# evoldoers/historian

Hardware: AMD Instinct MI355X
Metric: forward-DP cells/s (higher is better)
Workload: dtype f64; 1 GPU; batch of independent 2x2000-residue protein leaf-profile pairs, WAG, t=0.2/0.3, full (unbanded) Forward DP; scaled-probability recursion with the reference's truncation: every pairwise sum of the reference's left-nested log_sum_exp drops a term that is at most e^-10 of the other, as the reference's table does (src/logsumexp.h:45); no table, log-probabilities at the store; lpEnd within 1e-9 rel. of; pairs_per_gpu=512, pairs_total=512, parallelism=pairs farmed across 1 rank(s); RCCL broadcast of model constants only

## Files before the change

historian_amd/csrc/hx_linear.hip:

```cpp
#include <hip/hip_runtime.h>
#include <cstdlib>
#include "hx_device.h"
#include "hx_lse.h"
#include "hx_common.h"
#include "hx_policy.h"
#include "hx_kernels.h"

namespace hx {

namespace {

#define HXL_PUBLISH_LAG 16
#define HX_YL_MAX_CLS_LINEAR 64
#define HXL_EMIN (-(1 << 28))
#define HXL_RENORM_MASK 6

struct L5 { double imm, imd, idm, imi, iiw; int e; };

#define HXL_EXP_M10 4.5399929762484854e-05
__device__ __forceinline__ double trunc_sum(double a, double b) {
  const double hi = fmax_plain(a, b), lo = fmin_plain(a, b);
  const int keep = lo > hi * HXL_EXP_M10 ? __double2hiint(lo) : 0;
  return hi + __hiloint2double(keep, __double2loint(lo));
}
template <bool TRUNC> __device__ __forceinline__ double lin_acc(double m, double p, double acc) {
  if (TRUNC) return trunc_sum(acc, m * p);
  return __builtin_fma(m, p, acc);
}

__device__ __forceinline__ L5 l5_zero() { return L5{0., 0., 0., 0., 0., HXL_EMIN}; }

__device__ __forceinline__ int dpp_shr1_keep0(int old, int v) {
  return __builtin_amdgcn_update_dpp(old, v, 0x138, 0xf, 0xf, false);
}
__device__ __forceinline__ double dpp_shr1_keep0(double old, double v) {
  const int lo = __builtin_amdgcn_update_dpp(__double2loint(old), __double2loint(v), 0x138, 0xf, 0xf, false);
  const int hi = __builtin_amdgcn_update_dpp(__double2hiint(old), __double2hiint(v), 0x138, 0xf, 0xf, false);
  return __hiloint2double(hi, lo);
}
__device__ __forceinline__ L5 dpp_shr1_old(const L5& o, const L5& c) {
  return L5{dpp_shr1_keep0(o.imm, c.imm), dpp_shr1_keep0(o.imd, c.imd), dpp_shr1_keep0(o.idm, c.idm),
            dpp_shr1_keep0(o.imi, c.imi), dpp_shr1_keep0(o.iiw, c.iiw), dpp_shr1_keep0(o.e, c.e)};
}

#define HXL_LOG_ENTRIES 1536
typedef double log_entry __attribute__((ext_vector_type(2)));
__device__ __forceinline__ log_entry log_issue(double m, const HX_LDS double* ltab) {
  const double f = __builtin_amdgcn_frexp_mant(m);
  unsigned idx;
  asm("v_bfe_u32 %0, %1, 11, 11" : "=v"(idx) : "v"(__double2hiint(f)));
  return *(const HX_LDS log_entry*)((const HX_LDS char*)ltab + (idx << 4));
}
__device__ __forceinline__ double log_finish(double m, int e, log_entry ce) {
  const double f = __builtin_amdgcn_frexp_mant(m);
  const int k = __builtin_amdgcn_frexp_exp(m);
  const double r = __builtin_fma(f, ce.x, -1.0);
  double p = __builtin_fma(r, 1.0 / 3.0, -0.5);
  p = __builtin_fma(p, r, 1.0);
  const double lf = __builtin_fma(p, r, ce.y);
  return __builtin_fma((double)(e + k), 0.693147180559945309417, lf);
}
__device__ __forceinline__ double log_scaled(double m, int e, const HX_LDS double* ltab) { return log_finish(m, e, log_issue(m, ltab)); }

__device__ __forceinline__ L5 from_logs(double a, double b, double c, double d, double g) {
  const double mx = vmax(vmax(vmax(a, b), vmax(c, d)), g);
  if (!(mx > HX_NEG_INF)) return l5_zero();
  const double n = __builtin_rint(mx * 1.44269504088896340736);
  const double hi = n * 0.693147180369123816490, lo = n * 1.90821492927058770002e-10;
  L5 r;
  r.imm = exp((a - hi) - lo);
  r.imd = exp((b - hi) - lo);
  r.idm = exp((c - hi) - lo);
  r.imi = exp((d - hi) - lo);
  r.iiw = exp((g - hi) - lo);
  r.e = (int)n;
  return r;
}

struct LdsPlan { int elds, ycol, yclass, flags, zero;
                 int a0, b0, a1, stride, total; };

#define HXL_RING 64
#define HXL_STAGE 128

#define HXL_PATIENCE (1 << 22)
template <int W, bool BANDED, int PPW, int DIR, bool MULTI = false, bool TRUNC = false>
__global__ void __launch_bounds__(W * PPW * 64, 4)
k_fill_leaf_linear(const DevJob* __restrict__ jobs, const double* __restrict__ exact_tab, const double* __restrict__ log_tab,
                      const LdsPlan plan, const int n_jobs, const int groups = 1, int* const counters = nullptr) {
  static_assert(!MULTI || (!BANDED && PPW == 1 && W > 1), "several workgroups per pair: unbanded pairs, one pair per workgroup");
  static_assert(!BANDED || W == 1, "banded batches run one wavefront per pair");
  static_assert(PPW == 1 || BANDED, "several pairs per workgroup: banded batches only");
  constexpr int THREADS = W * PPW * 64, PT = W * 64;
  constexpr bool RESCHED = DIR == 0;
  constexpr int RING_ENTRIES = BANDED ? 0 : W * HXL_RING;
  typedef double d2v __attribute__((ext_vector_type(2)));
  extern __shared__ __attribute__((aligned(16))) unsigned char lds[];
  double* ltab = reinterpret_cast<double*>(lds);
  const int pair = PPW == 1 ? 0 : __builtin_amdgcn_readfirstlane((int)(threadIdx.x >> 6));
  const int tid = (int)threadIdx.x - pair * PT;
  const int G = MULTI ? groups : 1;
  const int job = MULTI ? (int)blockIdx.x / G : (int)blockIdx.x * PPW + pair;
  const int grp = MULTI ? (int)blockIdx.x % G : 0;
  const bool live = PPW == 1 || job < n_jobs;
  const DevJob& J = jobs[live ? job : 0];
  unsigned char* blk_a = lds + (pair == 0 ? plan.a0 : plan.a1 + (pair - 1) * plan.stride);
  unsigned char* blk_b = pair == 0 ? lds + plan.b0 : blk_a + (plan.stride - (RING_ENTRIES + HXL_STAGE) * 48);
  double* elds = reinterpret_cast<double*>(blk_a + plan.elds);
  unsigned* ycol = reinterpret_cast<unsigned*>(blk_a + plan.ycol);
  double* yclass = reinterpret_cast<double*>(blk_a + plan.yclass);
  volatile int* prog = reinterpret_cast<volatile int*>(blk_a + plan.flags);
  volatile int* cons = prog + W;
  volatile int* drain = cons + W;
  constexpr bool lds_words = !BANDED;
  for (int k = threadIdx.x; k < 2; k += THREADS) ltab[k] = log_tab[k];
  for (int k = 2048 + threadIdx.x; k < 2 * HXL_LOG_ENTRIES; k += THREADS) ltab[k] = log_tab[k];
  if (tid < 2 * W + 1) prog[tid] = 0;
  if (tid == 0) {
    d2v* z = reinterpret_cast<d2v*>(blk_a + plan.zero);
    z[0] = d2v{0., 0.}; z[1] = d2v{0., 0.}; z[2] = d2v{0., __hiloint2double(0, HXL_EMIN)};
  }
  {
    const int Ky1 = J.y.n_cls + 1, Kx1 = J.x.n_cls + 1;
    for (int jp = tid; jp < (lds_words ? J.n_cols + 130 : 0); jp += PT) {
      const int j = jp < 64 ? 0 : (jp - 64 >= J.n_cols ? J.n_cols - 1 : jp - 64);
      if (BANDED)
        ycol[jp] = (unsigned)J.y.ecls[j] | (J.y.pack[4 * (size_t)j + 3] < 0.0 ? 0x100u : 0u) |
                   ((J.y.flags[j] & F_EDGE) ? 0x200u : 0u) | (J.max_dist >= 0 ? (unsigned)J.y.env[j] << 10 : 0u);
      else if (DIR == 0)
        ycol[jp] = (unsigned)J.y.ecls[j] | (J.y.pack[4 * (size_t)j + 3] < 0.0 ? 0xFFFF0000u : 0u);
      else {
        const int jc = J.n_cols - 1 - j;
        ycol[jp] = (unsigned)J.y.ecls[jc + 1] | (J.y.pack[4 * (size_t)jc + 3] < 0.0 ? 0xFFFF0000u : 0u);
      }
    }
    for (int c = tid; c < Ky1; c += PT) {
      const bool real = c < J.y.n_cls;
      const int rep = real ? J.y.cls_rep[c] : 0;
      yclass[2 * c] = real ? exp(J.y.pack[4 * (size_t)rep + 1]) : 0.;
      yclass[2 * c + 1] = real ? exp(J.y.pack[4 * (size_t)rep + 2]) : 0.;
    }
    for (int e = tid; e < Kx1 * Ky1; e += PT) elds[e] = exp(J.emis_pad[e]);
  }
  __syncthreads();
  const int R = J.n_rows, Cc = J.n_cols;
  const int max_dist = J.max_dist;
  const int lane = threadIdx.x & 63, wave = PPW == 1 ? (RESCHED ? __builtin_amdgcn_readfirstlane((int)(threadIdx.x >> 6)) : (int)(threadIdx.x >> 6)) : 0;
  const int64_t plane = J.plane, ss = J.strip_stride;
  const int blk = J.blk;
  HX_GLOBAL double* __restrict__ M = as_global(DIR ? J.bwd : J.fwd);
  const HX_GLOBAL d4v* xpack = (const HX_GLOBAL d4v*)as_global(J.x.pack);
  double P[5][5];
#pragma unroll
  for (int a = 0; a < 5; ++a)
#pragma unroll
    for (int d = 0; d < 5; ++d) {
      const bool used = d == 0 || (d == 1 && a != 4) || (d == 2 && a != 3) || (d == 3 && (a == 0 || a == 3)) ||
                        (d == 4 && (a == 0 || a == 3 || a == 4));
      if (!used) { P[a][d] = 0.; continue; }
      const double pv = exp(J.T[a][d]);
      double v = __hiloint2double(__builtin_amdgcn_readfirstlane(__double2hiint(pv)), __builtin_amdgcn_readfirstlane(__double2loint(pv)));
      asm volatile("" : "+s"(v));
      P[a][d] = v;
    }
  volatile HX_LDS int* progp = (volatile HX_LDS int*)prog;
  volatile HX_LDS int* consp = (volatile HX_LDS int*)cons;
  volatile HX_LDS int* drainp = (volatile HX_LDS int*)drain;
  const HX_LDS double* lt = (const HX_LDS double*)ltab;
  HX_LDS d2v* ring_mine = (HX_LDS d2v*)blk_b + (size_t)wave * (HXL_RING * 3);
  const int n_strips = live ? (R + 63) / 64 : 0;
  const int prev_wave = (wave + W - 1) % W, next_wave = (wave + 1) % W;
  const int WT = W * G, gw = grp * W + wave;
  HX_GLOBAL int* gdrain = MULTI ? (HX_GLOBAL int*)as_global(counters + 256 * job) : nullptr;
  const int prev_grp = (grp + G - 1) % G;
  bool dead = false;
  const auto wait_drained = [&](const int need) {
    if (!MULTI) {
      while (drainp[0] < need) __builtin_amdgcn_s_sleep(1);
      asm volatile("" ::: "memory");
      return;
    }
    if (dead) return;
    int polls = 0;
    while (__builtin_amdgcn_readfirstlane(__hip_atomic_load(gdrain + prev_grp, __ATOMIC_RELAXED, __HIP_MEMORY_SCOPE_AGENT)) < need) {
      if (++polls > HXL_PATIENCE) {
        dead = true;
        if (lane == 0) __hip_atomic_store(gdrain + 255, 1, __ATOMIC_RELAXED, __HIP_MEMORY_SCOPE_AGENT);
        break;
      }
      __builtin_amdgcn_s_sleep(1);
    }
    asm volatile("" ::: "memory");
  };
  const auto publish_drained = [&](const int value) {
    if (lane != 0) return;
    if (MULTI) __hip_atomic_store(gdrain + grp, value, __ATOMIC_RELAXED, __HIP_MEMORY_SCOPE_AGENT);
    else drainp[0] = value;
  };
  HX_LDS d2v* staging = (HX_LDS d2v*)blk_b + (size_t)RING_ENTRIES * 3;
  const HX_LDS d2v* ring_prev = (const HX_LDS d2v*)blk_b + (size_t)prev_wave * (HXL_RING * 3);

  for (int s = gw; s < n_strips; s += WT) {
    const int row0 = s * 64;
    const int i0 = row0 + lane;
    const bool row_valid = i0 < R;
    double fx, f_imd, f_iiw;
    int x_wait;
    unsigned eoff;
    int env_x = 0;
    bool edge_x = true;
    {
      const int ic = row_valid ? (DIR ? R - 1 - i0 : i0) : 0;
      const d4v p = xpack[ic];
      const d4v q = DIR ? xpack[ic + 1] : p;
      fx = row_valid ? exp(q.x) : 0.;
      f_imd = row_valid ? exp(q.x + q.y) : 0.;
      f_iiw = row_valid ? exp(q.x + q.z) : 0.;
      x_wait = (row_valid && !(p.w < 0.0)) ? 0 : (1 << 29);
      eoff = (unsigned)J.x.ecls[DIR ? ic + 1 : ic] * (unsigned)(J.y.n_cls + 1);
      if (BANDED) {
        env_x = J.max_dist >= 0 ? J.x.env[ic] : 0;
        edge_x = (J.x.flags[ic] & F_EDGE) != 0 || J.max_dist < 0;
      }
    }
    L5 ca = l5_zero(), cb = l5_zero(), ua = l5_zero(), ub = l5_zero();
    const bool has_above = s > 0, has_below = s + 1 < n_strips;
    const bool wrap_in = has_above && wave == 0;
    const bool wrap_out = has_below && wave == W - 1;
    const bool ring_out = has_below && !wrap_out;
    const int above_base = ((s - 1) / WT) * Cc;
    const int my_base = (s / WT) * Cc;
    int64_t store_base = (int64_t)s * ss;
    int store_t0 = 0;
    const int nsteps = (Cc + 64) & ~1;

    auto wait_for = [&](const int cols) {
      const int need = above_base + (cols < Cc ? cols : Cc);
      while (progp[prev_wave] < need) __builtin_amdgcn_s_sleep(1);
      asm volatile("" ::: "memory");
    };
    const HX_LDS d2v* ring_above = !has_above ? (const HX_LDS d2v*)(blk_a + plan.zero) : wrap_in ? (const HX_LDS d2v*)staging : ring_prev;
    const int ring_base = (wrap_in || !has_above) ? 0 : above_base;
    const int ring_mask = !has_above ? 0 : wrap_in ? HXL_STAGE - 1 : HXL_RING - 1;
    auto ring_entry = [&](const int col) -> L5 {
      const HX_LDS d2v* q = ring_above + (size_t)((ring_base + col) & ring_mask) * 3;
      const d2v a = q[0], b = q[1], c = q[2];
      return L5{a.x, a.y, b.x, b.y, c.x, __double2loint(c.y)};
    };
    auto stage_block = [&](const int c0) {
      const int hi = (c0 + 64 < Cc) ? c0 + 64 : Cc;
      const int need = above_base + hi;
      wait_drained(need);
      const int jj = c0 + lane;
      const int64_t sl = jj < Cc ? ((BANDED && DIR == 0) ? stored_slot(J, row0 - 1, jj) : cell_slot_blk(ss, blk, row0 - 1, jj)) : -1;
      if (jj < Cc && sl < 0) {
        HX_LDS d2v* q = staging + (size_t)(jj & (HXL_STAGE - 1)) * 3;
        q[0] = d2v{0., 0.}; q[1] = d2v{0., 0.}; q[2] = d2v{0., __hiloint2double(0, HXL_EMIN)};
      }
      if (sl >= 0) {
        const double a = __hip_atomic_load(M + sl, __ATOMIC_RELAXED, __HIP_MEMORY_SCOPE_AGENT);
        const double b = __hip_atomic_load(M + plane + sl, __ATOMIC_RELAXED, __HIP_MEMORY_SCOPE_AGENT);
        const double c = __hip_atomic_load(M + 2 * plane + sl, __ATOMIC_RELAXED, __HIP_MEMORY_SCOPE_AGENT);
        const double d = __hip_atomic_load(M + 3 * plane + sl, __ATOMIC_RELAXED, __HIP_MEMORY_SCOPE_AGENT);
        const double g = __hip_atomic_load(M + 4 * plane + sl, __ATOMIC_RELAXED, __HIP_MEMORY_SCOPE_AGENT);
        L5 v = from_logs(a, b, c, d, g);
        if (BANDED && max_dist >= 0) {
          const int ia = DIR ? R - row0 : row0 - 1, ja = DIR ? Cc - 1 - jj : jj;
          int dist = J.x.env[ia] - J.y.env[ja];
          dist = dist < 0 ? -dist : dist;
          if (!(((J.x.flags[ia] | J.y.flags[ja]) & F_EDGE) || dist <= max_dist)) v = l5_zero();
        }
        HX_LDS d2v* q = staging + (size_t)(jj & (HXL_STAGE - 1)) * 3;
        q[0] = d2v{v.imm, v.imd};
        q[1] = d2v{v.idm, v.imi};
        q[2] = d2v{v.iiw, __hiloint2double(0, v.e)};
      }
      asm volatile("s_waitcnt lgkmcnt(0)" ::: "memory");
    };
    auto open_sweep = [&](const int t0) {
      if (!has_above) return;
      if (wrap_in) {
        if (t0 > 0 && (t0 & 63) == 0) stage_block(t0 - 64);
        if (t0 < Cc) stage_block(t0 & ~63);
      } else {
        wait_for(8);
      }
      const L5 b0 = ring_entry(t0), bd = ring_entry(t0 > 0 ? t0 - 1 : 0);
      if (lane == 0) {
        ua = b0;
        if (BANDED && t0 > 0) ub = bd;
      }
    };
    unsigned wnext = 0;
    const HX_GLOBAL unsigned* ywords = (const HX_GLOBAL unsigned*)as_global(DIR ? J.yword_bwd : J.yword);
    auto refill_words = [&](const int i0) {
      const unsigned v = ywords[i0 + lane];
      ycol[(i0 + lane) & 255] = v;
      asm volatile("s_waitcnt vmcnt(0) lgkmcnt(0)" ::: "memory");
    };
    auto first_words = [&](const int t0) {
      if (lds_words) { wnext = ycol[t0 + 64 - lane]; return; }
      refill_words(t0 & ~63); refill_words((t0 & ~63) + 64); refill_words((t0 & ~63) + 128);
      wnext = ycol[(t0 + 64 - lane) & 255];
    };
    auto next_word = [&](const int t) -> unsigned {
      const unsigned w = wnext;
      wnext = lds_words ? ycol[t + 65 - lane] : ycol[(t + 65 - lane) & 255];
      return w;
    };
    auto step = [&](const int t, const L5& left, L5& out, L5& u1, L5& u2, const unsigned w) {
      if (!lds_words && (t & 63) == 62) refill_words(t + 2 + 128);
      if ((t & 7) == 7 && has_above && t + 1 < Cc) {
        if (wrap_in) {
          if ((t & 63) == 63) stage_block(t + 1);
        } else {
          if (lane == 0) consp[wave] = above_base + t;
          wait_for(t + 9);
        }
      }
      const unsigned c = BANDED ? (w & 0xFFu) : (w & 0xFFFFu);
      const d2v rc = reinterpret_cast<const d2v*>(yclass)[c];
      const int y_wait = BANDED ? (int)((w & 0x100u) << 21) : (int)((w >> 16) << 13);
      const double em = elds[eoff + c];
      int E;
      if (DIR == 0) {
        double s_imm = u2.imm * P[0][0];
        s_imm = lin_acc<TRUNC>(u2.imd, P[1][0], s_imm);
        s_imm = lin_acc<TRUNC>(u2.idm, P[2][0], s_imm);
        s_imm = lin_acc<TRUNC>(u2.imi, P[3][0], s_imm);
        s_imm = lin_acc<TRUNC>(u2.iiw, P[4][0], s_imm);
        const int e_diag = u2.e;
        __builtin_amdgcn_sched_barrier(0);
        u2 = ring_entry(t + 1);
        __builtin_amdgcn_sched_barrier(0);
        double s_imd = u1.imm * P[0][1];
        double s_iiw = u1.imm * P[0][4];
        double s_idm = left.imm * P[0][2];
        double s_imi = left.imm * P[0][3];
        s_imd = lin_acc<TRUNC>(u1.imd, P[1][1], s_imd);
        s_iiw = lin_acc<TRUNC>(u1.imi, P[3][4], s_iiw);
        s_idm = lin_acc<TRUNC>(left.imd, P[1][2], s_idm);
        s_imi = lin_acc<TRUNC>(left.imi, P[3][3], s_imi);
        s_imd = lin_acc<TRUNC>(u1.idm, P[2][1], s_imd);
        s_iiw = lin_acc<TRUNC>(u1.iiw, P[4][4], s_iiw);
        s_idm = lin_acc<TRUNC>(left.idm, P[2][2], s_idm);
        s_imd = lin_acc<TRUNC>(u1.imi, P[3][1], s_imd);
        s_idm = lin_acc<TRUNC>(left.iiw, P[4][2], s_idm);
        E = left.e > u1.e ? left.e : u1.e;
        E = E > e_diag ? E : e_diag;
        int du = (u1.e - E) - y_wait, dl = (left.e - E) - x_wait, dd = e_diag - E;
        if (BANDED) {
          int dist = env_x - (int)(w >> 10);
          dist = dist < 0 ? -dist : dist;
          const int out_of_env = (edge_x || (w & 0x200u) || dist <= max_dist) ? 0 : (1 << 29);
          du -= out_of_env; dl -= out_of_env; dd -= out_of_env;
        }
        out.imd = __builtin_ldexp(s_imd * f_imd, du);
        out.iiw = __builtin_ldexp(s_iiw * f_iiw, du);
        out.idm = __builtin_ldexp(s_idm * rc.x, dl);
        out.imi = __builtin_ldexp(s_imi * rc.y, dl);
        out.imm = __builtin_ldexp(s_imm * (fx * em), dd);
      } else {
        const int e_diag = u2.e;
        const double tD = u2.imm * (fx * em);
        const double t1x = u1.imd * f_imd, t2x = u1.iiw * f_iiw;
        const double t1y = left.idm * rc.x, t2y = left.imi * rc.y;
        u2 = ring_entry(t + 1);
        E = left.e > u1.e ? left.e : u1.e;
        E = E > e_diag ? E : e_diag;
        int du = (u1.e - E) - y_wait, dl = (left.e - E) - x_wait, dd = e_diag - E;
        if (BANDED) {
          int dist = env_x - (int)(w >> 10);
          dist = dist < 0 ? -dist : dist;
          const int out_of_env = (edge_x || (w & 0x200u) || dist <= max_dist) ? 0 : (1 << 29);
          du -= out_of_env; dl -= out_of_env; dd -= out_of_env;
        }
        const double D = __builtin_ldexp(tD, dd);
        const double d1x = __builtin_ldexp(t1x, du), d2x = __builtin_ldexp(t2x, du);
        const double d1y = __builtin_ldexp(t1y, dl), d2y = __builtin_ldexp(t2y, dl);
        out.imm = lin_acc<TRUNC>(P[0][3], d2y, lin_acc<TRUNC>(P[0][2], d1y, lin_acc<TRUNC>(P[0][4], d2x, lin_acc<TRUNC>(P[0][1], d1x, P[0][0] * D))));
        out.imd = lin_acc<TRUNC>(P[1][2], d1y, lin_acc<TRUNC>(P[1][1], d1x, P[1][0] * D));
        out.idm = lin_acc<TRUNC>(P[2][2], d1y, lin_acc<TRUNC>(P[2][1], d1x, P[2][0] * D));
        out.imi = lin_acc<TRUNC>(P[3][3], d2y, lin_acc<TRUNC>(P[3][4], d2x, lin_acc<TRUNC>(P[3][1], d1x, P[3][0] * D)));
        out.iiw = lin_acc<TRUNC>(P[4][2], d1y, lin_acc<TRUNC>(P[4][4], d2x, P[4][0] * D));
      }
      out.e = E;
      if ((t & HXL_RENORM_MASK) == 0) {
        if (s == 0 && t == 0) {
          if (DIR == 0) {
            if (lane == 0) { out.imm = 1.0; out.e = 0; }
          } else if (lane == 0) {
            const double lpe = J.x.pack[4 * (size_t)R] + J.y.pack[4 * (size_t)Cc];
            out.imm = exp(lpe + J.T[0][5]); out.imd = exp(lpe + J.T[1][5]); out.idm = exp(lpe + J.T[2][5]);
            out.imi = exp(lpe + J.T[3][5]); out.iiw = exp(lpe + J.T[4][5]);
            out.e = 0;
          }
        }
        const double mx = vmax(vmax(vmax(out.imm, out.imd), vmax(out.idm, out.imi)), out.iiw);
        const int k = __builtin_amdgcn_frexp_exp(mx);
        out.imm = __builtin_ldexp(out.imm, -k);
        out.imd = __builtin_ldexp(out.imd, -k);
        out.idm = __builtin_ldexp(out.idm, -k);
        out.imi = __builtin_ldexp(out.imi, -k);
        out.iiw = __builtin_ldexp(out.iiw, -k);
        out.e = mx > 0. ? out.e + k : HXL_EMIN;
      }
      if (ring_out && t >= 63 && t - 63 < Cc) {
        const int col = t - 63;
        if ((col & 7) == 0) {
          const int need = my_base + col + 8 - HXL_RING;
          while (consp[next_wave] < need) __builtin_amdgcn_s_sleep(1);
          asm volatile("" ::: "memory");
        }
        if (lane == 63) {
          HX_LDS d2v* q = ring_mine + (size_t)((my_base + col) & (HXL_RING - 1)) * 3;
          q[0] = d2v{out.imm, out.imd};
          q[1] = d2v{out.idm, out.imi};
          q[2] = d2v{out.iiw, __hiloint2double(0, out.e)};
        }
        if ((col & 7) == 7 || col == Cc - 1) {
          asm volatile("" ::: "memory");
          if (lane == 63) progp[wave] = my_base + col + 1;
        }
      }
      u2 = dpp_shr1_old(u2, out);
    };

    int wlo[2] = {0, 0}, whi[2] = {nsteps, 0};
    if (BANDED) {
      const HX_GLOBAL int32_t* win = as_global(DIR ? J.bwd_windows : J.fwd_windows);
      if (win) {
        for (int w = 0; w < 2; ++w) {
          wlo[w] = win[4 * s + 2 * w] & ~1;
          const int h = (win[4 * s + 2 * w + 1] + 1) & ~1;
          whi[w] = h < nsteps ? h : nsteps;
        }
        if (whi[1] > wlo[1] && wlo[1] <= whi[0]) { whi[0] = whi[1] > whi[0] ? whi[1] : whi[0]; wlo[1] = whi[1] = 0; }
      }
    }
    for (int wi = 0; wi < (BANDED ? 2 : 1); ++wi) {
    if (BANDED && whi[wi] <= wlo[wi]) continue;
    const int wstart = BANDED ? wlo[wi] : 0, wend = BANDED ? whi[wi] : nsteps;
    if (BANDED) { ca = l5_zero(); cb = l5_zero(); ua = l5_zero(); ub = l5_zero(); }
    if (BANDED && DIR == 0 && J.strip_base) { store_base = J.strip_base[2 * s + wi]; store_t0 = wstart; }
    open_sweep(wstart);
    first_words(wstart);
    auto step_pair = [&](const int t) {
      if (RESCHED) {
        step(t, cb, ca, ua, ub, next_word(t));
        const log_entry ea0 = log_issue(ca.imm, lt), ea1 = log_issue(ca.imd, lt), ea2 = log_issue(ca.idm, lt),
                        ea3 = log_issue(ca.imi, lt), ea4 = log_issue(ca.iiw, lt);
        step(t + 1, ca, cb, ub, ua, next_word(t + 1));
        const log_entry eb0 = log_issue(cb.imm, lt), eb1 = log_issue(cb.imd, lt);
        __builtin_amdgcn_sched_barrier(0);
        const double l0 = log_finish(ca.imm, ca.e, ea0), l1 = log_finish(ca.imd, ca.e, ea1);
        const log_entry eb2 = log_issue(cb.idm, lt), eb3 = log_issue(cb.imi, lt);
        __builtin_amdgcn_sched_barrier(0);
        const double l2 = log_finish(ca.idm, ca.e, ea2), l3 = log_finish(ca.imi, ca.e, ea3);
        const log_entry eb4 = log_issue(cb.iiw, lt);
        __builtin_amdgcn_sched_barrier(0);
        const double l4 = log_finish(ca.iiw, ca.e, ea4);
        {
          HX_GLOBAL char* Mu = (HX_GLOBAL char*)(M + (store_base + (int64_t)((t - store_t0) >> 1) * blk));
          unsigned voff = (unsigned)lane << 4;
          asm("" : "+v"(voff));
          const int64_t pb = plane * 8;
          const auto put = [&](const int k, const double l, const double h) {
            const d2v v{l, h};
            if (MULTI) asm volatile("global_store_dwordx4 %0, %1, %2 sc1" ::"v"(voff), "v"(v), "s"(Mu + k * pb) : "memory");
            else __builtin_nontemporal_store(v, (HX_GLOBAL d2v*)(Mu + k * pb + voff));
          };
          const double h0 = log_finish(cb.imm, cb.e, eb0);
          put(0, l0, h0);
          const double h1 = log_finish(cb.imd, cb.e, eb1);
          put(1, l1, h1);
          const double h2 = log_finish(cb.idm, cb.e, eb2);
          put(2, l2, h2);
          const double h3 = log_finish(cb.imi, cb.e, eb3);
          put(3, l3, h3);
          const double h4 = log_finish(cb.iiw, cb.e, eb4);
          put(4, l4, h4);
        }
      } else {
        step(t, cb, ca, ua, ub, next_word(t));
        const double l0 = log_scaled(ca.imm, ca.e, lt), l1 = log_scaled(ca.imd, ca.e, lt),
                     l2 = log_scaled(ca.idm, ca.e, lt), l3 = log_scaled(ca.imi, ca.e, lt),
                     l4 = log_scaled(ca.iiw, ca.e, lt);
        step(t + 1, ca, cb, ub, ua, next_word(t + 1));
        const double h0 = log_scaled(cb.imm, cb.e, lt), h1 = log_scaled(cb.imd, cb.e, lt),
                     h2 = log_scaled(cb.idm, cb.e, lt), h3 = log_scaled(cb.imi, cb.e, lt),
                     h4 = log_scaled(cb.iiw, cb.e, lt);
        HX_GLOBAL d2v* M2 = (HX_GLOBAL d2v*)(M + (store_base + (lane << 1) + (int64_t)((t - store_t0) >> 1) * blk));
        const int64_t plane2 = plane >> 1;
        if (MULTI) {
          const d2v v0{l0, h0}, v1{l1, h1}, v2{l2, h2}, v3{l3, h3}, v4{l4, h4};
          asm volatile("global_store_dwordx4 %0, %1, off sc1" ::"v"(&M2[0]), "v"(v0) : "memory");
          asm volatile("global_store_dwordx4 %0, %1, off sc1" ::"v"(&M2[plane2]), "v"(v1) : "memory");
          asm volatile("global_store_dwordx4 %0, %1, off sc1" ::"v"(&M2[2 * plane2]), "v"(v2) : "memory");
          asm volatile("global_store_dwordx4 %0, %1, off sc1" ::"v"(&M2[3 * plane2]), "v"(v3) : "memory");
          asm volatile("global_store_dwordx4 %0, %1, off sc1" ::"v"(&M2[4 * plane2]), "v"(v4) : "memory");
        } else {
          __builtin_nontemporal_store(d2v{l0, h0}, &M2[0]);
          __builtin_nontemporal_store(d2v{l1, h1}, &M2[plane2]);
          __builtin_nontemporal_store(d2v{l2, h2}, &M2[2 * plane2]);
          __builtin_nontemporal_store(d2v{l3, h3}, &M2[3 * plane2]);
          __builtin_nontemporal_store(d2v{l4, h4}, &M2[4 * plane2]);
        }
      }
      if (wrap_out && !BANDED) {
        const int fin = (t + 2 < nsteps ? t + 2 : nsteps) - 63;
        if (fin >= Cc) {
          asm volatile("s_waitcnt vmcnt(0)" ::: "memory");
          publish_drained(my_base + Cc);
        } else {
          const int done = fin - HXL_PUBLISH_LAG;
          if (done > 0 && ((done >> 6) != ((done - 2) >> 6))) {
            constexpr int PUBLISH_WAIT = 5 * (HXL_PUBLISH_LAG / 2);
            static_assert(PUBLISH_WAIT <= 63 && HXL_PUBLISH_LAG % 2 == 0, "s_waitcnt vmcnt holds 6 bits");
            asm volatile("s_waitcnt vmcnt(%0)" ::"n"(PUBLISH_WAIT) : "memory");
            publish_drained(my_base + done);
          }
        }
      }
    };
    for (int t = wstart; t < wend; t += 2) step_pair(t);
    }
    if (BANDED && wrap_out) {
      asm volatile("s_waitcnt vmcnt(0)" ::: "memory");
      publish_drained(my_base + Cc);
    }
    if (has_above && !wrap_in && lane == 0) consp[wave] = above_base + Cc;
    if (MULTI && s == n_strips - 1) {
      asm volatile("s_waitcnt vmcnt(0)" ::: "memory");
      __builtin_amdgcn_fence(__ATOMIC_ACQUIRE, "agent");
      asm volatile("s_waitcnt vmcnt(0)" ::: "memory");
      const bool gave_up = __hip_atomic_load(gdrain + 255, __ATOMIC_RELAXED, __HIP_MEMORY_SCOPE_AGENT) != 0;
      if (lane == 0) {
        if (DIR == 0) *J.lp_end = gave_up ? __builtin_nan("") : forward_lp_end(J, ExactLse{exact_tab});
        else *J.lp_start = gave_up ? __builtin_nan("") : J.bwd[cell_slot_blk(ss, blk, R - 1, Cc - 1)];
      }
    }
  }
  if (MULTI) return;
  asm volatile("s_waitcnt vmcnt(0)" ::: "memory");
  __syncthreads();
  if (live && wave == 0 && lane == 0) {
    if (DIR == 0) *J.lp_end = forward_lp_end(J, ExactLse{exact_tab});
    else *J.lp_start = J.bwd[cell_slot_blk(ss, blk, R - 1, Cc - 1)];
  }
}

}

int log_table_doubles() { return 2 * HXL_LOG_ENTRIES; }
void build_log_table(double* out) {
  for (int k = 0; k < 2 * HXL_LOG_ENTRIES; ++k) out[k] = 0.;
  out[1] = -HUGE_VAL;
  for (int k = 0; k < 512; ++k) {
    const double centre = 0.5 * (1.0 + (k + 0.5) / 512.0);
    const double c = 1.0 / centre;
    out[2 * (1024 + k)] = c;
    out[2 * (1024 + k) + 1] = -log(c);
  }
}

static LdsPlan plan_lds(int W, int PPW, bool banded, int yl_cols, int yl_emis, int yl_cls) {
  LdsPlan p;
  const int table = 16 * HXL_LOG_ENTRIES, hole = 16 * 1024;
  int a = 0;
  p.elds = a; a += (8 * yl_emis + 15) & ~15;
  p.ycol = a; a += banded ? 4 * 256 : (4 * (yl_cols + 132) + 15) & ~15;
  p.yclass = a; a += 16 * yl_cls;
  p.flags = a; a += (4 * (2 * W + 1) + 15) & ~15;
  p.zero = a; a += 48;
  const int b = ((banded ? 0 : W * HXL_RING) + HXL_STAGE) * 48;
  int end = table;
  if (16 + a + b <= hole) { p.a0 = 16; p.b0 = 16 + a; }
  else if (16 + a <= hole) { p.a0 = 16; p.b0 = end; end += b; }
  else { p.a0 = end; p.b0 = end + a; end += a + b; }
  p.a1 = end;
  p.stride = a + b;
  end += (PPW - 1) * p.stride;
  p.total = (end + 15) & ~15;
  return p;
}

int launch_forward_leaf_linear(const DevJob* d_jobs, int n_jobs, int max_rows, bool banded, Tab8 tab8, Tab16 tab16,
                               int yl_cols, int yl_emis, int yl_cls, int multi, int* counters, bool trunc, hipStream_t st) {
  const double* tab = tab8.p;
  const double* log_tab = tab16.p;
  if (yl_cls > HX_YL_MAX_CLS_LINEAR + 1) return launch_fail("%d emission classes exceed the scaled-probability kernel's column words", yl_cls);
  if (multi > 1 && !banded) {
    const LdsPlan p = plan_lds(4, 1, false, yl_cols, yl_emis, yl_cls);
    if (p.total > HX_LDS_LIMIT) return launch_fail("k_fill_leaf_linear<multi> needs %d bytes of LDS (limit %d)", p.total, HX_LDS_LIMIT);
    if (trunc)
      hipLaunchKernelGGL((k_fill_leaf_linear<4, false, 1, 0, true, true>), dim3(n_jobs * multi), dim3(4 * 64), p.total, st, d_jobs, tab, log_tab, p, n_jobs,
                         multi, counters);
    else
      hipLaunchKernelGGL((k_fill_leaf_linear<4, false, 1, 0, true>), dim3(n_jobs * multi), dim3(4 * 64), p.total, st, d_jobs, tab, log_tab, p, n_jobs,
                         multi, counters);
    return 0;
  }
#define HXL_LAUNCH(W_, B_, PPW_) do { const LdsPlan p = plan_lds(W_, PPW_, B_, yl_cols, yl_emis, yl_cls); \
    if (p.total > HX_LDS_LIMIT) return launch_fail("k_fill_leaf_linear<%d> needs %d bytes of LDS (limit %d)", W_, p.total, HX_LDS_LIMIT); \
    if (trunc) hipLaunchKernelGGL((k_fill_leaf_linear<W_, B_, PPW_, 0, false, true>), dim3((n_jobs + PPW_ - 1) / PPW_), dim3(W_ * PPW_ * 64), p.total, st, \
                       d_jobs, tab, log_tab, p, n_jobs); \
    else hipLaunchKernelGGL((k_fill_leaf_linear<W_, B_, PPW_, 0>), dim3((n_jobs + PPW_ - 1) / PPW_), dim3(W_ * PPW_ * 64), p.total, st, \
                       d_jobs, tab, log_tab, p, n_jobs); } while (0)
  if (banded) {
    const char* v = getenv("HX_LINEAR_PPW");
    const int forced = v ? atoi(v) : 0;
    if (forced > 1 || (forced == 0 && n_jobs > 1024)) {
      if (plan_lds(1, 6, true, yl_cols, yl_emis, yl_cls).total <= 76 * 1024) HXL_LAUNCH(1, true, 6);
      else if (plan_lds(1, 5, true, yl_cols, yl_emis, yl_cls).total <= 76 * 1024) HXL_LAUNCH(1, true, 5);
      else HXL_LAUNCH(1, true, 4);
    } else HXL_LAUNCH(1, true, 1);
    return 0;
  }
  const char* v = getenv("HX_LINEAR_WAVES");
  const int forced = v ? atoi(v) : 0;
  if (forced == 1) HXL_LAUNCH(1, false, 1);
  else if (forced == 2) HXL_LAUNCH(2, false, 1);
  else if (forced == 4) HXL_LAUNCH(4, false, 1);
  else if (forced == 8) HXL_LAUNCH(8, false, 1);
  else if (forced == 16) HXL_LAUNCH(16, false, 1);
  else if (max_rows <= 64) HXL_LAUNCH(1, false, 1);
  else if (max_rows <= 128) HXL_LAUNCH(2, false, 1);
  else if (max_rows <= 256) HXL_LAUNCH(4, false, 1);
  else if (max_rows <= 512 || n_jobs > 256) HXL_LAUNCH(8, false, 1);
  else HXL_LAUNCH(16, false, 1);
#undef HXL_LAUNCH
  return 0;
}

int launch_backward_leaf_linear(const DevJob* d_jobs, int n_jobs, int max_rows, bool banded, Tab8 tab8, Tab16 tab16,
                                int yl_cols, int yl_emis, int yl_cls, int multi, int* counters, bool trunc, hipStream_t st) {
  const double* tab = tab8.p;
  const double* log_tab = tab16.p;
  if (yl_cls > HX_YL_MAX_CLS_LINEAR + 1) return launch_fail("%d emission classes exceed the scaled-probability kernel's column words", yl_cls);
  if (multi > 1 && !banded) {
    const LdsPlan p = plan_lds(4, 1, false, yl_cols, yl_emis, yl_cls);
    if (p.total > HX_LDS_LIMIT) return launch_fail("k_fill_leaf_linear<multi> needs %d bytes of LDS (limit %d)", p.total, HX_LDS_LIMIT);
    if (trunc)
      hipLaunchKernelGGL((k_fill_leaf_linear<4, false, 1, 1, true, true>), dim3(n_jobs * multi), dim3(4 * 64), p.total, st, d_jobs, tab, log_tab, p, n_jobs,
                         multi, counters);
    else
      hipLaunchKernelGGL((k_fill_leaf_linear<4, false, 1, 1, true>), dim3(n_jobs * multi), dim3(4 * 64), p.total, st, d_jobs, tab, log_tab, p, n_jobs,
                         multi, counters);
    return 0;
  }
#define HXL_LAUNCH(W_, B_, PPW_) do { const LdsPlan p = plan_lds(W_, PPW_, B_, yl_cols, yl_emis, yl_cls); \
    if (p.total > HX_LDS_LIMIT) return launch_fail("k_fill_leaf_linear<%d, bwd> needs %d bytes of LDS (limit %d)", W_, p.total, HX_LDS_LIMIT); \
    if (trunc) hipLaunchKernelGGL((k_fill_leaf_linear<W_, B_, PPW_, 1, false, true>), dim3((n_jobs + PPW_ - 1) / PPW_), dim3(W_ * PPW_ * 64), p.total, st, \
                       d_jobs, tab, log_tab, p, n_jobs); \
    else hipLaunchKernelGGL((k_fill_leaf_linear<W_, B_, PPW_, 1>), dim3((n_jobs + PPW_ - 1) / PPW_), dim3(W_ * PPW_ * 64), p.total, st, \
                       d_jobs, tab, log_tab, p, n_jobs); } while (0)
  if (banded) {
    const char* v = getenv("HX_LINEAR_PPW");
    const int forced = v ? atoi(v) : 0;
    if (forced > 1 || (forced == 0 && n_jobs > 1024)) {
      if (plan_lds(1, 6, true, yl_cols, yl_emis, yl_cls).total <= 76 * 1024) HXL_LAUNCH(1, true, 6);
      else if (plan_lds(1, 5, true, yl_cols, yl_emis, yl_cls).total <= 76 * 1024) HXL_LAUNCH(1, true, 5);
      else HXL_LAUNCH(1, true, 4);
    } else HXL_LAUNCH(1, true, 1);
    return 0;
  }
  const char* v = getenv("HX_LINEAR_WAVES");
  const int forced = v ? atoi(v) : 0;
  if (forced == 1) HXL_LAUNCH(1, false, 1);
  else if (forced == 2) HXL_LAUNCH(2, false, 1);
  else if (forced == 8) HXL_LAUNCH(8, false, 1);
  else if (max_rows <= 64) HXL_LAUNCH(1, false, 1);
  else if (max_rows <= 128) HXL_LAUNCH(2, false, 1);
  else if (max_rows <= 256) HXL_LAUNCH(4, false, 1);
  else if (max_rows <= 512 || n_jobs > 256) HXL_LAUNCH(8, false, 1);
  else HXL_LAUNCH(16, false, 1);
#undef HXL_LAUNCH
  return 0;
}

}
```

Measured before the change: 114.0 billion cells/s.

## Hand off pre-contracted upper-row sums through ring in forward DP

In the forward direction, each cell now computes the transition-weighted sums its lower neighbours need (diag imm, vertical imd and iiw) right after it is produced. It passes only those three values plus the exponent through the DPP shift and the LDS ring, instead of all five states. This moves the upper-row contractions out of the critical step, shrinks ring traffic and register pressure, and cuts cross-lane DPP moves from six to four. Staged rows read from global memory are contracted the same way. Separately, the final log FMA takes ln2 as a scalar operand through inline asm.

```diff
diff --git a/historian_amd/csrc/hx_linear.hip b/historian_amd/csrc/hx_linear.hip
--- a/historian_amd/csrc/hx_linear.hip
+++ b/historian_amd/csrc/hx_linear.hip
@@ -16,6 +16,10 @@
 #define HXL_RENORM_MASK 6
 
 struct L5 { double imm, imd, idm, imi, iiw; int e; };
+struct H3 { double imm, imd, iiw; int e; };
+template <int DIR> struct HandOff { typedef L5 type; };
+template <> struct HandOff<0> { typedef H3 type; };
+typedef double d2v __attribute__((ext_vector_type(2)));
 
 #define HXL_EXP_M10 4.5399929762484854e-05
 __device__ __forceinline__ double trunc_sum(double a, double b) {
@@ -29,6 +33,9 @@
 }
 
 __device__ __forceinline__ L5 l5_zero() { return L5{0., 0., 0., 0., 0., HXL_EMIN}; }
+template <class T> __device__ __forceinline__ T hand_off_zero();
+template <> __device__ __forceinline__ L5 hand_off_zero<L5>() { return l5_zero(); }
+template <> __device__ __forceinline__ H3 hand_off_zero<H3>() { return H3{0., 0., 0., HXL_EMIN}; }
 
 __device__ __forceinline__ int dpp_shr1_keep0(int old, int v) {
   return __builtin_amdgcn_update_dpp(old, v, 0x138, 0xf, 0xf, false);
@@ -41,6 +48,26 @@
 __device__ __forceinline__ L5 dpp_shr1_old(const L5& o, const L5& c) {
   return L5{dpp_shr1_keep0(o.imm, c.imm), dpp_shr1_keep0(o.imd, c.imd), dpp_shr1_keep0(o.idm, c.idm),
             dpp_shr1_keep0(o.imi, c.imi), dpp_shr1_keep0(o.iiw, c.iiw), dpp_shr1_keep0(o.e, c.e)};
+}
+__device__ __forceinline__ H3 dpp_shr1_old(const H3& o, const H3& c) {
+  return H3{dpp_shr1_keep0(o.imm, c.imm), dpp_shr1_keep0(o.imd, c.imd), dpp_shr1_keep0(o.iiw, c.iiw), dpp_shr1_keep0(o.e, c.e)};
+}
+__device__ __forceinline__ void ring_put(HX_LDS d2v* q, const L5& v) {
+  q[0] = d2v{v.imm, v.imd};
+  q[1] = d2v{v.idm, v.imi};
+  q[2] = d2v{v.iiw, __hiloint2double(0, v.e)};
+}
+__device__ __forceinline__ void ring_put(HX_LDS d2v* q, const H3& v) {
+  q[0] = d2v{v.imm, v.imd};
+  q[1] = d2v{v.iiw, __hiloint2double(0, v.e)};
+}
+__device__ __forceinline__ void ring_get(const HX_LDS d2v* q, L5& v) {
+  const d2v a = q[0], b = q[1], c = q[2];
+  v = L5{a.x, a.y, b.x, b.y, c.x, __double2loint(c.y)};
+}
+__device__ __forceinline__ void ring_get(const HX_LDS d2v* q, H3& v) {
+  const d2v a = q[0], b = q[1];
+  v = H3{a.x, a.y, b.x, __double2loint(b.y)};
 }
 
 #define HXL_LOG_ENTRIES 1536
@@ -51,6 +78,7 @@
   asm("v_bfe_u32 %0, %1, 11, 11" : "=v"(idx) : "v"(__double2hiint(f)));
   return *(const HX_LDS log_entry*)((const HX_LDS char*)ltab + (idx << 4));
 }
+template <bool FMA3 = false>
 __device__ __forceinline__ double log_finish(double m, int e, log_entry ce) {
   const double f = __builtin_amdgcn_frexp_mant(m);
   const int k = __builtin_amdgcn_frexp_exp(m);
@@ -58,7 +86,13 @@
   double p = __builtin_fma(r, 1.0 / 3.0, -0.5);
   p = __builtin_fma(p, r, 1.0);
   const double lf = __builtin_fma(p, r, ce.y);
-  return __builtin_fma((double)(e + k), 0.693147180559945309417, lf);
+  const double kd = (double)(e + k), ln2 = 0.693147180559945309417;
+  if (FMA3) {
+    double res;
+    asm("v_fma_f64 %0, %1, %2, %3" : "=v"(res) : "v"(kd), "s"(ln2), "v"(lf));
+    return res;
+  }
+  return __builtin_fma(kd, ln2, lf);
 }
 __device__ __forceinline__ double log_scaled(double m, int e, const HX_LDS double* ltab) { return log_finish(m, e, log_issue(m, ltab)); }
 
@@ -94,7 +128,7 @@
   constexpr int THREADS = W * PPW * 64, PT = W * 64;
   constexpr bool RESCHED = DIR == 0;
   constexpr int RING_ENTRIES = BANDED ? 0 : W * HXL_RING;
-  typedef double d2v __attribute__((ext_vector_type(2)));
+  typedef typename HandOff<DIR>::type HO;
   extern __shared__ __attribute__((aligned(16))) unsigned char lds[];
   double* ltab = reinterpret_cast<double*>(lds);
   const int pair = PPW == 1 ? 0 : __builtin_amdgcn_readfirstlane((int)(threadIdx.x >> 6));
@@ -116,10 +150,6 @@
   for (int k = threadIdx.x; k < 2; k += THREADS) ltab[k] = log_tab[k];
   for (int k = 2048 + threadIdx.x; k < 2 * HXL_LOG_ENTRIES; k += THREADS) ltab[k] = log_tab[k];
   if (tid < 2 * W + 1) prog[tid] = 0;
-  if (tid == 0) {
-    d2v* z = reinterpret_cast<d2v*>(blk_a + plan.zero);
-    z[0] = d2v{0., 0.}; z[1] = d2v{0., 0.}; z[2] = d2v{0., __hiloint2double(0, HXL_EMIN)};
-  }
   {
     const int Ky1 = J.y.n_cls + 1, Kx1 = J.x.n_cls + 1;
     for (int jp = tid; jp < (lds_words ? J.n_cols + 130 : 0); jp += PT) {
@@ -163,6 +193,29 @@
       asm volatile("" : "+s"(v));
       P[a][d] = v;
     }
+  const auto hand_off = [&](const L5& c) -> HO {
+    if constexpr (DIR == 0) {
+      H3 h;
+      h.imm = c.imm * P[0][0];
+      h.imm = lin_acc<TRUNC>(c.imd, P[1][0], h.imm);
+      h.imm = lin_acc<TRUNC>(c.idm, P[2][0], h.imm);
+      h.imm = lin_acc<TRUNC>(c.imi, P[3][0], h.imm);
+      h.imm = lin_acc<TRUNC>(c.iiw, P[4][0], h.imm);
+      h.imd = c.imm * P[0][1];
+      h.iiw = c.imm * P[0][4];
+      h.imd = lin_acc<TRUNC>(c.imd, P[1][1], h.imd);
+      h.iiw = lin_acc<TRUNC>(c.imi, P[3][4], h.iiw);
+      h.imd = lin_acc<TRUNC>(c.idm, P[2][1], h.imd);
+      h.iiw = lin_acc<TRUNC>(c.iiw, P[4][4], h.iiw);
+      h.imd = lin_acc<TRUNC>(c.imi, P[3][1], h.imd);
+      h.e = c.e;
+      return h;
+    } else {
+      return c;
+    }
+  };
+  HX_LDS d2v* zero_entry = (HX_LDS d2v*)(blk_a + plan.zero);
+  if (tid == 0) ring_put(zero_entry, hand_off(l5_zero()));
   volatile HX_LDS int* progp = (volatile HX_LDS int*)prog;
   volatile HX_LDS int* consp = (volatile HX_LDS int*)cons;
   volatile HX_LDS int* drainp = (volatile HX_LDS int*)drain;
@@ -223,7 +276,8 @@
         edge_x = (J.x.flags[ic] & F_EDGE) != 0 || J.max_dist < 0;
       }
     }
-    L5 ca = l5_zero(), cb = l5_zero(), ua = l5_zero(), ub = l5_zero();
+    L5 ca = l5_zero(), cb = l5_zero();
+    HO ua = hand_off_zero<HO>(), ub = hand_off_zero<HO>();
     const bool has_above = s > 0, has_below = s + 1 < n_strips;
     const bool wrap_in = has_above && wave == 0;
     const bool wrap_out = has_below && wave == W - 1;
@@ -239,13 +293,13 @@
       while (progp[prev_wave] < need) __builtin_amdgcn_s_sleep(1);
       asm volatile("" ::: "memory");
     };
-    const HX_LDS d2v* ring_above = !has_above ? (const HX_LDS d2v*)(blk_a + plan.zero) : wrap_in ? (const HX_LDS d2v*)staging : ring_prev;
+    const HX_LDS d2v* ring_above = !has_above ? (const HX_LDS d2v*)zero_entry : wrap_in ? (const HX_LDS d2v*)staging : ring_prev;
     const int ring_base = (wrap_in || !has_above) ? 0 : above_base;
     const int ring_mask = !has_above ? 0 : wrap_in ? HXL_STAGE - 1 : HXL_RING - 1;
-    auto ring_entry = [&](const int col) -> L5 {
-      const HX_LDS d2v* q = ring_above + (size_t)((ring_base + col) & ring_mask) * 3;
-      const d2v a = q[0], b = q[1], c = q[2];
-      return L5{a.x, a.y, b.x, b.y, c.x, __double2loint(c.y)};
+    auto ring_entry = [&](const int col) -> HO {
+      HO v;
+      ring_get(ring_above + (size_t)((ring_base + col) & ring_mask) * 3, v);
+      return v;
     };
     auto stage_block = [&](const int c0) {
       const int hi = (c0 + 64 < Cc) ? c0 + 64 : Cc;
@@ -254,8 +308,9 @@
       const int jj = c0 + lane;
       const int64_t sl = jj < Cc ? ((BANDED && DIR == 0) ? stored_slot(J, row0 - 1, jj) : cell_slot_blk(ss, blk, row0 - 1, jj)) : -1;
       if (jj < Cc && sl < 0) {
-        HX_LDS d2v* q = staging + (size_t)(jj & (HXL_STAGE - 1)) * 3;
-        q[0] = d2v{0., 0.}; q[1] = d2v{0., 0.}; q[2] = d2v{0., __hiloint2double(0, HXL_EMIN)};
+        HO z;
+        ring_get(zero_entry, z);
+        ring_put(staging + (size_t)(jj & (HXL_STAGE - 1)) * 3, z);
       }
       if (sl >= 0) {
         const double a = __hip_atomic_load(M + sl, __ATOMIC_RELAXED, __HIP_MEMORY_SCOPE_AGENT);
@@ -270,10 +325,8 @@
           dist = dist < 0 ? -dist : dist;
           if (!(((J.x.flags[ia] | J.y.flags[ja]) & F_EDGE) || dist <= max_dist)) v = l5_zero();
         }
-        HX_LDS d2v* q = staging + (size_t)(jj & (HXL_STAGE - 1)) * 3;
-        q[0] = d2v{v.imm, v.imd};
-        q[1] = d2v{v.idm, v.imi};
-        q[2] = d2v{v.iiw, __hiloint2double(0, v.e)};
+        if (DIR == 0) asm("" : "+v"(v.imm), "+v"(v.imd), "+v"(v.idm), "+v"(v.imi), "+v"(v.iiw));
+        ring_put(staging + (size_t)(jj & (HXL_STAGE - 1)) * 3, hand_off(v));
       }
       asm volatile("s_waitcnt lgkmcnt(0)" ::: "memory");
     };
@@ -285,7 +338,7 @@
       } else {
         wait_for(8);
       }
-      const L5 b0 = ring_entry(t0), bd = ring_entry(t0 > 0 ? t0 - 1 : 0);
+      const HO b0 = ring_entry(t0), bd = ring_entry(t0 > 0 ? t0 - 1 : 0);
       if (lane == 0) {
         ua = b0;
         if (BANDED && t0 > 0) ub = bd;
@@ -308,7 +361,7 @@
       wnext = lds_words ? ycol[t + 65 - lane] : ycol[(t + 65 - lane) & 255];
       return w;
     };
-    auto step = [&](const int t, const L5& left, L5& out, L5& u1, L5& u2, const unsigned w) {
+    auto step = [&](const int t, const L5& left, L5& out, HO& u1, HO& u2, const unsigned w) {
       if (!lds_words && (t & 63) == 62) refill_words(t + 2 + 128);
       if ((t & 7) == 7 && has_above && t + 1 < Cc) {
         if (wrap_in) {
@@ -323,28 +376,18 @@
       const int y_wait = BANDED ? (int)((w & 0x100u) << 21) : (int)((w >> 16) << 13);
       const double em = elds[eoff + c];
       int E;
-      if (DIR == 0) {
-        double s_imm = u2.imm * P[0][0];
-        s_imm = lin_acc<TRUNC>(u2.imd, P[1][0], s_imm);
-        s_imm = lin_acc<TRUNC>(u2.idm, P[2][0], s_imm);
-        s_imm = lin_acc<TRUNC>(u2.imi, P[3][0], s_imm);
-        s_imm = lin_acc<TRUNC>(u2.iiw, P[4][0], s_imm);
+      if constexpr (DIR == 0) {
+        const double s_imm = u2.imm;
         const int e_diag = u2.e;
         __builtin_amdgcn_sched_barrier(0);
         u2 = ring_entry(t + 1);
         __builtin_amdgcn_sched_barrier(0);
-        double s_imd = u1.imm * P[0][1];
-        double s_iiw = u1.imm * P[0][4];
+        const double s_imd = u1.imd, s_iiw = u1.iiw;
         double s_idm = left.imm * P[0][2];
         double s_imi = left.imm * P[0][3];
-        s_imd = lin_acc<TRUNC>(u1.imd, P[1][1], s_imd);
-        s_iiw = lin_acc<TRUNC>(u1.imi, P[3][4], s_iiw);
         s_idm = lin_acc<TRUNC>(left.imd, P[1][2], s_idm);
         s_imi = lin_acc<TRUNC>(left.imi, P[3][3], s_imi);
-        s_imd = lin_acc<TRUNC>(u1.idm, P[2][1], s_imd);
-        s_iiw = lin_acc<TRUNC>(u1.iiw, P[4][4], s_iiw);
         s_idm = lin_acc<TRUNC>(left.idm, P[2][2], s_idm);
-        s_imd = lin_acc<TRUNC>(u1.imi, P[3][1], s_imd);
         s_idm = lin_acc<TRUNC>(left.iiw, P[4][2], s_idm);
         E = left.e > u1.e ? left.e : u1.e;
         E = E > e_diag ? E : e_diag;
@@ -405,6 +448,7 @@
         out.iiw = __builtin_ldexp(out.iiw, -k);
         out.e = mx > 0. ? out.e + k : HXL_EMIN;
       }
+      const HO o = hand_off(out);
       if (ring_out && t >= 63 && t - 63 < Cc) {
         const int col = t - 63;
         if ((col & 7) == 0) {
@@ -412,18 +456,13 @@
           while (consp[next_wave] < need) __builtin_amdgcn_s_sleep(1);
           asm volatile("" ::: "memory");
         }
-        if (lane == 63) {
-          HX_LDS d2v* q = ring_mine + (size_t)((my_base + col) & (HXL_RING - 1)) * 3;
-          q[0] = d2v{out.imm, out.imd};
-          q[1] = d2v{out.idm, out.imi};
-          q[2] = d2v{out.iiw, __hiloint2double(0, out.e)};
-        }
+        if (lane == 63) ring_put(ring_mine + (size_t)((my_base + col) & (HXL_RING - 1)) * 3, o);
         if ((col & 7) == 7 || col == Cc - 1) {
           asm volatile("" ::: "memory");
           if (lane == 63) progp[wave] = my_base + col + 1;
         }
       }
-      u2 = dpp_shr1_old(u2, out);
+      u2 = dpp_shr1_old(u2, o);
     };
 
     int wlo[2] = {0, 0}, whi[2] = {nsteps, 0};
@@ -441,7 +480,7 @@
     for (int wi = 0; wi < (BANDED ? 2 : 1); ++wi) {
     if (BANDED && whi[wi] <= wlo[wi]) continue;
     const int wstart = BANDED ? wlo[wi] : 0, wend = BANDED ? whi[wi] : nsteps;
-    if (BANDED) { ca = l5_zero(); cb = l5_zero(); ua = l5_zero(); ub = l5_zero(); }
+    if (BANDED) { ca = l5_zero(); cb = l5_zero(); ua = hand_off_zero<HO>(); ub = hand_off_zero<HO>(); }
     if (BANDED && DIR == 0 && J.strip_base) { store_base = J.strip_base[2 * s + wi]; store_t0 = wstart; }
     open_sweep(wstart);
     first_words(wstart);
@@ -453,13 +492,13 @@
         step(t + 1, ca, cb, ub, ua, next_word(t + 1));
         const log_entry eb0 = log_issue(cb.imm, lt), eb1 = log_issue(cb.imd, lt);
         __builtin_amdgcn_sched_barrier(0);
-        const double l0 = log_finish(ca.imm, ca.e, ea0), l1 = log_finish(ca.imd, ca.e, ea1);
+        const double l0 = log_finish<true>(ca.imm, ca.e, ea0), l1 = log_finish<true>(ca.imd, ca.e, ea1);
         const log_entry eb2 = log_issue(cb.idm, lt), eb3 = log_issue(cb.imi, lt);
         __builtin_amdgcn_sched_barrier(0);
-        const double l2 = log_finish(ca.idm, ca.e, ea2), l3 = log_finish(ca.imi, ca.e, ea3);
+        const double l2 = log_finish<true>(ca.idm, ca.e, ea2), l3 = log_finish<true>(ca.imi, ca.e, ea3);
         const log_entry eb4 = log_issue(cb.iiw, lt);
         __builtin_amdgcn_sched_barrier(0);
-        const double l4 = log_finish(ca.iiw, ca.e, ea4);
+        const double l4 = log_finish<true>(ca.iiw, ca.e, ea4);
         {
           HX_GLOBAL char* Mu = (HX_GLOBAL char*)(M + (store_base + (int64_t)((t - store_t0) >> 1) * blk));
           unsigned voff = (unsigned)lane << 4;
@@ -470,15 +509,15 @@
             if (MULTI) asm volatile("global_store_dwordx4 %0, %1, %2 sc1" ::"v"(voff), "v"(v), "s"(Mu + k * pb) : "memory");
             else __builtin_nontemporal_store(v, (HX_GLOBAL d2v*)(Mu + k * pb + voff));
           };
-          const double h0 = log_finish(cb.imm, cb.e, eb0);
+          const double h0 = log_finish<true>(cb.imm, cb.e, eb0);
           put(0, l0, h0);
-          const double h1 = log_finish(cb.imd, cb.e, eb1);
+          const double h1 = log_finish<true>(cb.imd, cb.e, eb1);
           put(1, l1, h1);
-          const double h2 = log_finish(cb.idm, cb.e, eb2);
+          const double h2 = log_finish<true>(cb.idm, cb.e, eb2);
           put(2, l2, h2);
-          const double h3 = log_finish(cb.imi, cb.e, eb3);
+          const double h3 = log_finish<true>(cb.imi, cb.e, eb3);
           put(3, l3, h3);
-          const double h4 = log_finish(cb.iiw, cb.e, eb4);
+          const double h4 = log_finish<true>(cb.iiw, cb.e, eb4);
           put(4, l4, h4);
         }
       } else {
```

After: 114.8 billion cells/s, median of 6. About the same (+0.7%).
